# Ansh4121/audio-deepfake-detection-fmsl

Hardware: NVIDIA B200
Metric: utterances/sec (4 s, 16 kHz) LFCC+delta+delta-delta front-end (higher is better)
Workload: dtype f32 (split-fp16 tensor-core DFT, fp32 accumulate)

## Files before the change

### audio-deepfake-detection-fmsl_b200/csrc/fe_gemm_tables.h

```cpp
#ifndef FE_GEMM_TABLES_H_
#define FE_GEMM_TABLES_H_
#include "fe_common.h"

int64_t fe_gemm_plan_layout(const b200fe_params* p, fe_blob_header* h, int64_t off);
int32_t fe_gemm_pack(const b200fe_params* p, fe_blob_header* h, const float* window,
                     const float* fbank, char* base);
bool fe_gemm_variant_built(void);
bool fe_gemm_auto_prefers(const b200fe_params* p);
#endif
```

### audio-deepfake-detection-fmsl_b200/csrc/fe_stream.cu

```cuda
#include <atomic>
#include <stdio.h>
#include <unistd.h>

#include "fe_tc.cuh"

#include "fe_gemm.cuh"
#include "fe_gemm.h"
#include "fe_gemm_tables.h"

namespace {

constexpr int kDrainWarps = 16;
constexpr int kProducerWarp0 = kDrainWarps;
constexpr int kProducerGroups = 2;
constexpr int kProducerWarps = 4 * kProducerGroups;
constexpr int kProducerThreads = kProducerWarps * 32;
constexpr int kMmaWarp0 = kProducerWarp0 + kProducerWarps;
constexpr int kNumMmaWarps = 2;
constexpr int kLoaderWarp = kMmaWarp0 + kNumMmaWarps;
constexpr int kThreads = (kLoaderWarp + 1) * 32;
constexpr int kTileM = FE_GEMM_TILE_M;
constexpr int kMaxSlots = 131;
constexpr int kAStageBytes = 8 * 2 * kTileM * 16;
constexpr int kGmaxStride = (((kMaxSlots + 1) * 4 + 15) & ~15) / 4;

struct stream_args {
  const float* wave;
  const void* tables;
  float* energies;
  unsigned int* group_max;
  int* error_flag;
  int64_t T;
  int64_t row_base;
  int32_t rows, n_frames, n_filter, hop, nhalf, nstages, kpairs;
  int32_t total_frames, tile_frames, n_tiles, top_db_group;
  const int64_t* offsets;
  const int32_t* lengths;
  int64_t flat_rel, dense_rel;
};

__device__ __forceinline__ int64_t row_src(const stream_args& a, int row) {
  if (!a.offsets) return (int64_t)row * a.T;
  const int64_t arow = a.row_base + row;
  const int64_t off = __ldg(a.offsets + arow);
  return fe_clip_in_place(off, __ldg(a.lengths + arow), a.T, a.flat_rel) ? a.flat_rel + off : a.dense_rel + (int64_t)row * a.T;
}

constexpr int kNumBars = 14;

struct smem_layout {
  int samp, a_stage, b_stage, dw, dwn, dctl, dhdr, mid, gmax, us2, midp, exl0, exch, bars, tmem_slot, total;
};

__host__ __device__ inline smem_layout make_layout(int hop, int nhalf, int kpairs) {
  smem_layout L;
  int off = 0;
  L.samp = off;      off += kMaxSlots * hop * 4;
  off = (off + 127) & ~127;
  L.a_stage = off;   off += 2 * kAStageBytes;
  L.b_stage = off;   off += 2 * fe_gemm_b_stage_bytes(nhalf);
  L.dw = off;        off += 2 * (nhalf / 2) * (int)sizeof(fe_drain_w);
  L.dwn = off;       off += 2 * (nhalf / FE_DRAIN_BATCH) * 16 * 4;
  L.dctl = off;      off += (2 * (nhalf / FE_DRAIN_BATCH) * 4 + 15) & ~15;
  L.dhdr = off;      off += (int)sizeof(fe_drain_hdr);
  L.mid = off;       off += kpairs * 4;
  L.gmax = off;      off += 2 * (((kMaxSlots + 1) * 4 + 15) & ~15);
  L.us2 = off;       off += 2 * kTileM * 4;
  L.midp = off;      off += 2 * kProducerGroups * kTileM * 8;
  L.exl0 = off;      off += 2 * 2 * 2 * kTileM * 4;
  L.exch = off;      off += 2 * 2 * kTileM * 4;
  L.bars = off;      off += kNumBars * 8;
  L.tmem_slot = off; off += 16;
  L.total = off;
  return L;
}

enum { BAR_SAMP_FULL = 0, BAR_SAMP_EMPTY = 1, BAR_A_FULL = 2, BAR_B_FULL = 4, BAR_STAGE_FREE = 6, BAR_ACC_FULL = 8,
       BAR_ACC_EMPTY = 9, BAR_PROD_DONE = 10, BAR_SCOUT_FULL = 12, BAR_COUNT = 14 };
static_assert(BAR_COUNT == kNumBars, "barrier count");

#ifdef FE_GEMM_TRACE
#ifndef FE_TRACE_CTA
#define FE_TRACE_CTA 0
#endif
#ifndef FE_TRACE_IT0
#define FE_TRACE_IT0 0
#endif
#define ST_TRACE(ev, it, q) do { if (blockIdx.x == FE_TRACE_CTA && (int)(it) >= FE_TRACE_IT0 && (int)(it) < FE_TRACE_IT0 + 8) { ((long long*)(a.error_flag + 64))[(((int)(it) - FE_TRACE_IT0) * 8 + (q)) * 16 + (ev)] = clock64(); } } while (0)
#else
#define ST_TRACE(ev, it, q) do { } while (0)
#endif

__device__ __forceinline__ uint32_t swz(uint32_t o) { return o ^ (((o >> 7) & 7u) << 4); }

struct tmaps8 {
  CUtensorMap m[8];
};

__device__ __forceinline__ void tma_box_4d(uint32_t dst, const CUtensorMap* map, uint32_t bar, int c0, int c1, int c2, int c3) {
  asm volatile(
      "cp.async.bulk.tensor.4d.shared::cluster.global.mbarrier::complete_tx::bytes [%0], [%1, {%3, %4, %5, %6}], [%2];" ::"r"(dst),
      "l"(map), "r"(bar), "r"(c0), "r"(c1), "r"(c2), "r"(c3)
      : "memory");
}

__device__ __forceinline__ void tma_box_5d(uint32_t dst, const CUtensorMap* map, uint32_t bar, int c0, int c1, int c2, int c3, int c4) {
  asm volatile(
      "cp.async.bulk.tensor.5d.shared::cluster.global.mbarrier::complete_tx::bytes [%0], [%1, {%3, %4, %5, %6, %7}], [%2];" ::"r"(dst),
      "l"(map), "r"(bar), "r"(c0), "r"(c1), "r"(c2), "r"(c3), "r"(c4)
      : "memory");
}
// ... 106 lines not shown
    tmem_ld8(t0 + 2 * tn, se);
    tmem_ld8(t0 + 3 * tn, so);
#endif
    tmem_ld_wait();
    tmem_ld_tie8(ce); tmem_ld_tie8(co); tmem_ld_tie8(se); tmem_ld_tie8(so);
    unsigned ctl;
    asm volatile("ld.shared.u32 %0, [%1];" : "=r"(ctl) : "r"(ctl_addr));
    fe_drain_w w[4];
#pragma unroll
    for (int p = 0; p < 4; ++p)
      asm volatile("ld.shared.v4.f32 {%0, %1, %2, %3}, [%4];" : "=f"(w[p].w[0][0]), "=f"(w[p].w[0][1]), "=f"(w[p].w[1][0]), "=f"(w[p].w[1][1])
                   : "r"(w_addr + 16u * p));
    if (left == 1) {
      tc_fence_before();
      __syncwarp();
      if (lane == 0) mbar_arrive(acc_empty_bar);
    }
    fe_f2 pw[4];
#ifdef FE_EXP_NO_MATH
    st.acc[0].x += ce[0] + co[1] + se[2] + so[3];
    continue;
#endif
#pragma unroll
    for (int p = 0; p < 4; ++p)
      pw[p] = fe_drain_power<RUN>(fe_f2{ce[2 * p], ce[2 * p + 1]}, fe_f2{co[2 * p], co[2 * p + 1]}, fe_f2{se[2 * p], se[2 * p + 1]},
                                  fe_f2{so[2 * p], so[2 * p + 1]});
    fe_drain_batch(pw, w, reinterpret_cast<const float*>(__cvta_shared_to_generic(wn_addr)), ctl, st, emit);
  }
}


// ... 11 lines not shown
    asm volatile("ld.shared.v4.f32 {%0, %1, %2, %3}, [%4];" : "=f"(b.x), "=f"(b.y), "=f"(b.z), "=f"(b.w)
                 : "r"(smem_u32(s_samp) + swz(brow + (hop - j0 - 16) * 4 + ch * 16)));
    buf[4 * ch + 0] = b.x; buf[4 * ch + 1] = b.y; buf[4 * ch + 2] = b.z; buf[4 * ch + 3] = b.w;
  }
  bwd[0] = (j0 == 0) ? fwd[0] : *reinterpret_cast<const float*>(s_samp + swz(brow + (hop - j0) * 4));
#pragma unroll
  for (int i = 1; i < 16; ++i) bwd[i] = buf[16 - i];
  fe_u4 chunk[8];
  fe_stream_produce_unit(fwd, bwd, scale, s_mid + j0, mid_re, mid_im, chunk);
  mbar_wait(bar_stage_free, free_parity, error_flag, 7);
  unsigned char* a_row = a_slot + khalf * kTileM * 16 + m * 16;
#pragma unroll
  for (int sf = 0; sf < 8; ++sf) *reinterpret_cast<fe_u4*>(a_row + sf * fe_gemm_tile_bytes(kTileM)) = chunk[sf];
  fence_proxy_async();
  __syncwarp();
  if (lane == 0) mbar_arrive(bar_a_full);
}

__global__ void __launch_bounds__(kThreads, 1) fe_stream_kernel(const __grid_constant__ tmaps8 maps, const stream_args a) {
  extern __shared__ __align__(1024) unsigned char smem[];
  const smem_layout L = make_layout(a.hop, a.nhalf, a.kpairs);
  const int tid = threadIdx.x, warp = tid >> 5, lane = tid & 31;
  const unsigned char* blob = reinterpret_cast<const unsigned char*>(a.tables);
  const fe_blob_header* h = reinterpret_cast<const fe_blob_header*>(blob);
  const int nF = a.n_frames, hop = a.hop, nfil = a.n_filter;
  const int rs = hop * 4;
  const int npairs = a.nhalf / 2, nbatch = a.nhalf / FE_DRAIN_BATCH;

  if (!h->gemm_ok) {
    if (tid == 0) mbar_timeout(a.error_flag, 98);
    return;
  }
  unsigned char* s_samp = smem + L.samp;
  fe_drain_w* s_dw = reinterpret_cast<fe_drain_w*>(smem + L.dw);
  uint32_t* s_dctl = reinterpret_cast<uint32_t*>(smem + L.dctl);
  float* s_dwn = reinterpret_cast<float*>(smem + L.dwn);
  fe_drain_hdr* s_dhdr = reinterpret_cast<fe_drain_hdr*>(smem + L.dhdr);
  float* s_mid = reinterpret_cast<float*>(smem + L.mid);
  float* s_gmax = reinterpret_cast<float*>(smem + L.gmax);
  float* s_us2 = reinterpret_cast<float*>(smem + L.us2);
  float2* s_midp = reinterpret_cast<float2*>(smem + L.midp);
  float* s_exl0 = reinterpret_cast<float*>(smem + L.exl0);
  float* s_exch = reinterpret_cast<float*>(smem + L.exch);
  uint32_t* s_tmem = reinterpret_cast<uint32_t*>(smem + L.tmem_slot);
  const uint32_t bars = smem_u32(smem + L.bars);
  auto bar = [&](int i) { return bars + 8u * (uint32_t)i; };

  {
    const fe_drain_w* gdw = reinterpret_cast<const fe_drain_w*>(blob + h->off_gemm_dw);
    for (int i = tid; i < 2 * npairs; i += kThreads) s_dw[i] = gdw[i];
    const uint32_t* gctl = reinterpret_cast<const uint32_t*>(blob + h->off_gemm_dctl);
    for (int i = tid; i < 2 * nbatch; i += kThreads) s_dctl[i] = gctl[i];
    const float* gwn = reinterpret_cast<const float*>(blob + h->off_gemm_dwn);
    for (int i = tid; i < 2 * nbatch * 16; i += kThreads) s_dwn[i] = gwn[i];
    const int32_t* ghdr = reinterpret_cast<const int32_t*>(blob + h->off_gemm_dids);
    for (int i = tid; i < (int)(sizeof(fe_drain_hdr) / 4); i += kThreads) reinterpret_cast<int32_t*>(s_dhdr)[i] = ghdr[i];
    const float* gmid = reinterpret_cast<const float*>(blob + h->off_gemm_mid);
    for (int i = tid; i < a.kpairs; i += kThreads) s_mid[i] = (i & 1) ? gmid[a.kpairs + i] : gmid[i];
    float4* z = reinterpret_cast<float4*>(s_samp);
    for (int i = tid; i < kMaxSlots * rs / 16; i += kThreads) z[i] = make_float4(0.f, 0.f, 0.f, 0.f);
    fence_proxy_async();
  }
  if (tid == 0) {
    mbar_init(bar(BAR_SAMP_FULL), 2);
    mbar_init(bar(BAR_SAMP_EMPTY), kProducerWarps);
    mbar_init(bar(BAR_A_FULL + 0), 8);
    mbar_init(bar(BAR_A_FULL + 1), 8);
    mbar_init(bar(BAR_B_FULL + 0), 1);
    mbar_init(bar(BAR_B_FULL + 1), 1);
    mbar_init(bar(BAR_STAGE_FREE + 0), kNumMmaWarps);
    mbar_init(bar(BAR_STAGE_FREE + 1), kNumMmaWarps);
    mbar_init(bar(BAR_ACC_FULL), kNumMmaWarps);
    mbar_init(bar(BAR_ACC_EMPTY), kDrainWarps);
    mbar_init(bar(BAR_PROD_DONE + 0), kProducerWarps);
    mbar_init(bar(BAR_PROD_DONE + 1), kProducerWarps);
    mbar_init(bar(BAR_SCOUT_FULL + 0), kDrainWarps);
    mbar_init(bar(BAR_SCOUT_FULL + 1), kDrainWarps);
    asm volatile("fence.mbarrier_init.release.cluster;" ::: "memory");
  }
  if (warp == kMmaWarp0) {
    asm volatile("tcgen05.alloc.cta_group::1.sync.aligned.shared::cta.b32 [%0], %1;" ::"r"(smem_u32(s_tmem)), "r"(512));
    asm volatile("tcgen05.relinquish_alloc_permit.cta_group::1.sync.aligned;" ::);
  }
  tc_fence_before();
  __syncthreads();
  tc_fence_after();
  const uint32_t tmem_base = *s_tmem;
  const int T = (int)a.T;
  const uint32_t b_stage_bytes = (uint32_t)fe_gemm_b_stage_bytes(a.nhalf);

  if (warp == kLoaderWarp) {
    const unsigned char* gB = blob + h->off_gemm_b;
    const uint32_t row_bytes = (uint32_t)hop * 4u;
    uint32_t n = 0, it = 0;
    for (int tile = blockIdx.x; tile < a.n_tiles; tile += gridDim.x, ++it) {
      const fe_tile_geo g = fe_tile_geometry(tile, a.tile_frames, a.total_frames, nF);
      mbar_wait_relaxed(bar(BAR_SAMP_EMPTY), (it & 1u) ^ 1u, a.error_flag, 1);
      ST_TRACE(0, it, 0);
      int n_edge = 0;
      for (int row = g.row0; row <= g.row_last; ++row) {
        const int sa = row * (nF + 1) - g.sv0, sb = sa + nF;
        n_edge += (sa >= 0 && sa < g.nv) + (sb >= 0 && sb < g.nv);
      }
      fence_proxy_async();
      if (lane == 0) mbar_arrive_expect_tx(bar(BAR_SAMP_FULL), (uint32_t)(g.nv - n_edge) * row_bytes);
      __syncwarp();
      for (int row = g.row0; row <= g.row_last; ++row) {
        const int v_lo = max(g.sv0 - row * (nF + 1), 1), v_hi = min(g.sv0 + g.nv - 1 - row * (nF + 1), nF - 1);
        const int cnt = v_hi - v_lo + 1;
        if (cnt <= 0) continue;
        if (lane < 8 && ((cnt >> lane) & 1)) {
// ... 30 lines not shown
      if (tile + (int)gridDim.x < a.n_tiles) {
        const fe_tile_geo gn = fe_tile_geometry(tile + gridDim.x, a.tile_frames, a.total_frames, nF);
        for (int row = gn.row0; row <= gn.row_last; ++row) {
          const int v_lo = max(gn.sv0 - row * (nF + 1), 1), v_hi = min(gn.sv0 + gn.nv - 1 - row * (nF + 1), nF - 1);
          const int cnt = v_hi - v_lo + 1;
          if (cnt <= 0) continue;
          if (lane < 8 && ((cnt >> lane) & 1)) {
            const int first = cnt & ~((2 << lane) - 1);
            row_prefetch(a, &maps.m[lane], v_lo - 1 + first, row);
          }
        }
      }
      if (lane == 0) {
        for (int q = 0; q < a.nstages; ++q, ++n) {
          const uint32_t s = n & 1u, par = (n >> 1) & 1u;
          mbar_wait_relaxed(bar(BAR_STAGE_FREE + s), par ^ 1u, a.error_flag, 2);
          mbar_arrive_expect_tx(bar(BAR_B_FULL + s), b_stage_bytes);
          bulk_g2s(smem_u32(smem + L.b_stage + s * b_stage_bytes), gB + (size_t)q * b_stage_bytes, b_stage_bytes,
                   bar(BAR_B_FULL + s));
        }
      }
      __syncwarp();
    }
  } else if (warp >= kMmaWarp0) {
    {
      const int sub0 = (4 / kNumMmaWarps) * __shfl_sync(0xffffffffu, warp - kMmaWarp0, 0);
      const uint32_t tmem_u = __shfl_sync(0xffffffffu, tmem_base, 0);
      const uint32_t idesc = (1u << 4) | ((uint32_t)(a.nhalf >> 3) << 17) | ((uint32_t)(kTileM >> 4) << 24);
      const uint32_t b_lbo = (uint32_t)a.nhalf * 16u;
      const uint32_t smem_a = smem_u32(smem + L.a_stage), smem_b = smem_u32(smem + L.b_stage);
      const uint32_t tile_bytes_a = fe_gemm_tile_bytes(kTileM), tile_bytes_b = fe_gemm_tile_bytes(a.nhalf);
      uint32_t n = 0, it = 0;
      for (int tile = blockIdx.x; tile < a.n_tiles; tile += gridDim.x, ++it) {
        mbar_wait_relaxed(bar(BAR_ACC_EMPTY), (it & 1u) ^ 1u, a.error_flag, 3);
        tc_fence_after();
        if (sub0 == 0 && lane == 0) ST_TRACE(8, it, 0);
        for (int q = 0; q < a.nstages; ++q, ++n) {
          const uint32_t s = n & 1u, par = (n >> 1) & 1u;
          mbar_wait_relaxed(bar(BAR_B_FULL + s), par, a.error_flag, 4);
          if (sub0 == 0 && lane == 0) ST_TRACE(10, it, q);
          mbar_wait_relaxed(bar(BAR_A_FULL + s), par, a.error_flag, 5);
          tc_fence_after();
          if (sub0 == 0 && lane == 0) ST_TRACE(3, it, q);
          const uint32_t a_base = smem_a + s * kAStageBytes;
          const uint32_t b_base = smem_b + s * b_stage_bytes;
          if (elect_one()) {
#ifdef FE_EXP_TWO_PRODUCTS
            constexpr int kProducts = 2;
#else
            constexpr int kProducts = 3;
#endif
#pragma unroll
            for (int pr = 0; pr < kProducts; ++pr) {
#pragma unroll
              for (int ds = 0; ds < 4 / kNumMmaWarps; ++ds) {
                const int sub = sub0 + ds;
                const uint64_t da = make_desc(a_base + (2 * sub + (pr == 1 ? 1 : 0)) * tile_bytes_a, kTileM * 16, 128);
                const uint64_t db = make_desc(b_base + (2 * sub + (pr == 2 ? 1 : 0)) * tile_bytes_b, b_lbo, 128);
                umma_f16(tmem_u + (uint32_t)(sub * a.nhalf), da, db, idesc, (q > 0 || pr > 0) ? 1u : 0u);
              }
            }
            umma_commit(bar(BAR_STAGE_FREE + s));
            if (q == a.nstages - 1) umma_commit(bar(BAR_ACC_FULL));
          }
          __syncwarp();
        }
      }
    }
  } else if (warp >= kProducerWarp0) {
    const int pw = warp - kProducerWarp0;
    const int grp = pw >> 2;
    const int quarter = pw & 3;
    const int m = quarter * 32 + lane;
    uint32_t n0 = 0, it = 0;
    for (int tile = blockIdx.x; tile < a.n_tiles; tile += gridDim.x, ++it, n0 += (uint32_t)a.nstages) {
      const fe_tile_geo g = fe_tile_geometry(tile, a.tile_frames, a.total_frames, nF);
      const int mm = min(m, g.count - 1);
      const int row = (g.g0 + mm) / nF;
      const int slot = mm + (row - g.row0);
      const uint32_t tp = it & 1u;
      mbar_wait(bar(BAR_SCOUT_FULL + tp), (it >> 1) & 1u, a.error_flag, 10);
      float scale, unscale;
      {
        const float* gm = s_gmax + tp * kGmaxStride;
        fe_gemm_frame_scale(2.0f * fmaxf(gm[slot], gm[slot + 1]), scale, unscale);
      }
      mbar_wait(bar(BAR_SAMP_FULL), tp, a.error_flag, 6);
      if (tid == kProducerWarp0 * 32) ST_TRACE(1, it, 0);
      if (grp == 0) s_us2[tp * kTileM + m] = unscale * unscale;
      const uint32_t brow = (uint32_t)(slot * rs), frow = brow + (uint32_t)rs;
      float mid_re = 0.0f, mid_im = 0.0f;
#pragma unroll 1
      for (int q = 0; q < a.nstages; ++q) {
        const uint32_t n = n0 + (uint32_t)q, sl = n & 1u, par = (n >> 1) & 1u;
        produce_unit(s_samp, brow, frow, hop, q, grp, m, scale, s_mid, mid_re, mid_im, smem + L.a_stage + sl * kAStageBytes,
                     bar(BAR_STAGE_FREE + sl), par ^ 1u, bar(BAR_A_FULL + sl), a.error_flag, lane);
        if (lane == 0 && quarter == 0) ST_TRACE(2, it, q);
      }
      s_midp[(tp * kProducerGroups + grp) * kTileM + m] = make_float2(mid_re, mid_im);
      __syncwarp();
      if (lane == 0) {
        mbar_arrive(bar(BAR_SAMP_EMPTY));
        mbar_arrive(bar(BAR_PROD_DONE + tp));
      }
    }
  } else {
    const int quarter = warp & 3;
    const int run = (warp >> 2) & 1;
    const int half = warp >> 3;
    const int m = quarter * 32 + lane;
    const fe_drain_w* w_run = s_dw + run * npairs;
    const uint32_t* ctl_run = s_dctl + run * nbatch;
    const float* wn_run = s_dwn + run * nbatch * 16;
    const uint32_t tbase = tmem_base + ((uint32_t)(quarter * 32) << 16);
    const int k_begin = half * (a.nhalf >> 1), k_end = k_begin + (a.nhalf >> 1);
    for (int pre = 0; pre < 2; ++pre) {
      const int tile = blockIdx.x + pre * gridDim.x;
      if (tile < a.n_tiles) {
        const fe_tile_geo g = fe_tile_geometry(tile, a.tile_frames, a.total_frames, nF);
        scout_tile_global(a, nF, hop, g, s_gmax + pre * kGmaxStride, warp, kDrainWarps, lane);
      }
      __syncwarp();
      if (lane == 0) mbar_arrive(bar(BAR_SCOUT_FULL + pre));
    }
    uint32_t it = 0;
    for (int tile = blockIdx.x; tile < a.n_tiles; tile += gridDim.x, ++it) {
      const fe_tile_geo g = fe_tile_geometry(tile, a.tile_frames, a.total_frames, nF);
      const int mm = min(m, g.count - 1);
      const int row = (g.g0 + mm) / nF;
      const int t = (g.g0 + mm) - row * nF;
      const uint32_t tp = it & 1u;
      mbar_wait(bar(BAR_PROD_DONE + tp), (it >> 1) & 1u, a.error_flag, 9);
      emit_store emit;
      emit.base = a.energies;
      emit.off = (uint32_t)((row * nfil) * nF + t);
      emit.n_frames = (uint32_t)nF;
      emit.n_filter = nfil;
      emit.valid = m < g.count;
      emit.us2 = s_us2[tp * kTileM + m];
      emit.vmax = 0.0f;
      float p_mid = 0.0f;
      if (run == 0 && half == 1) {
        const float2 v0 = s_midp[(tp * kProducerGroups + 0) * kTileM + m], v1 = s_midp[(tp * kProducerGroups + 1) * kTileM + m];
        const float bs = (float)(1 << FE_GEMM_B_SCALE_LOG2);
        const float re = (v0.x + v1.x) * bs, im = (v0.y + v1.y) * bs;
        p_mid = fmaf(re, re, im * im);
      }
      fe_drain_state st;
      fe_drain_init(st, *s_dhdr, run, half);
      mbar_wait(bar(BAR_ACC_FULL), tp, a.error_flag, 8);
      tc_fence_after();
      if (lane == 0 && quarter == 0) ST_TRACE(4, it, warp >> 2);
      if (run == 0) drain_walk<0>(tbase, a.nhalf, k_begin, k_end, w_run, ctl_run, wn_run, st, emit, bar(BAR_ACC_EMPTY), lane);
      else drain_walk<1>(tbase, a.nhalf, k_begin, k_end, w_run, ctl_run, wn_run, st, emit, bar(BAR_ACC_EMPTY), lane);
      if (lane == 0 && quarter == 0) ST_TRACE(5, it, warp >> 2);
      float* l0p = s_exl0 + ((tp * 2 + run) * 2) * kTileM + m;
      if (half == 0) {
        l0p[0] = fe_drain_leftover(st, 0, 0.0f, 0.0f);
        l0p[kTileM] = fe_drain_leftover(st, 1, 0.0f, 0.0f);
        quarter_bar(quarter);
      } else {
        quarter_bar(quarter);
        const float l0[2] = {l0p[0], l0p[kTileM]};
        float left[2];
        fe_drain_join_halves(st, *s_dhdr, run, l0, p_mid, left, emit);
        float* ex = s_exch + tp * 2 * kTileM + m;
        if (run == 1) {
          if (s_dhdr->merge[0]) ex[0] = left[0]; else emit(s_dhdr->last[1][0], left[0]);
          if (s_dhdr->merge[1]) ex[kTileM] = left[1]; else emit(s_dhdr->last[1][1], left[1]);
          runs_bar(quarter);
        } else {
          runs_bar(quarter);
          emit(s_dhdr->last[0][0], s_dhdr->merge[0] ? left[0] + ex[0] : left[0]);
          emit(s_dhdr->last[0][1], s_dhdr->merge[1] ? left[1] + ex[kTileM] : left[1]);
        }
      }
      if (a.group_max) {
        const int grp_id = (int)((a.row_base + row) / a.top_db_group);
        const int grp0 = __shfl_sync(0xffffffffu, grp_id, 0);
        if (__all_sync(0xffffffffu, grp_id == grp0)) {
          const unsigned wmax = __reduce_max_sync(0xffffffffu, __float_as_uint(emit.vmax));
          if (lane == 0) atomicMax(a.group_max + grp0, wmax);
        } else if (emit.valid) {
          atomicMax(a.group_max + grp_id, __float_as_uint(emit.vmax));
        }
      }
      if (lane == 0 && quarter == 0) ST_TRACE(6, it, warp >> 2);
      {
        const int tile2 = tile + 2 * (int)gridDim.x;
        if (tile2 < a.n_tiles) {
          const fe_tile_geo g2 = fe_tile_geometry(tile2, a.tile_frames, a.total_frames, nF);
          scout_tile_global(a, nF, hop, g2, s_gmax + tp * kGmaxStride, warp, kDrainWarps, lane);
        }
        __syncwarp();
        if (lane == 0) mbar_arrive(bar(BAR_SCOUT_FULL + tp));
        if (lane == 0 && quarter == 0) ST_TRACE(7, it, warp >> 2);
      }
    }
  }

  tc_fence_before();
  __syncthreads();
  if (warp == kMmaWarp0) {
    asm volatile("tcgen05.dealloc.cta_group::1.sync.aligned.b32 %0, %1;" ::"r"(tmem_base), "r"(512));
  }
}

typedef CUresult (*encode_tiled_fn)(CUtensorMap*, CUtensorMapDataType, cuuint32_t, void*, const cuuint64_t*,
                                    const cuuint64_t*, const cuuint32_t*, const cuuint32_t*, CUtensorMapInterleave,
                                    CUtensorMapSwizzle, CUtensorMapL2promotion, CUtensorMapFloatOOBfill);

encode_tiled_fn get_encode() {
  static std::atomic<encode_tiled_fn> cached{nullptr};
  encode_tiled_fn fn = cached.load(std::memory_order_relaxed);
  if (!fn) {
    void* p = nullptr;
    cudaDriverEntryPointQueryResult q;
    if (cudaGetDriverEntryPoint("cuTensorMapEncodeTiled", &p, cudaEnableDefault, &q) == cudaSuccess &&
        q == cudaDriverEntryPointSuccess) {
      fn = (encode_tiled_fn)p;
      cached.store(fn, std::memory_order_relaxed);
    }
  }
  return fn;
}

}

#ifdef FE_GEMM_TRACE
int* fe_trace_host_flag = nullptr;
#endif
int32_t fe_gemm_compiled(void) { return 1; }

bool fe_gemm_supported(const b200fe_params* p) {
  if (p->n_filter < 1 || p->n_filter > FE_GEMM_MAX_FILTERS) return false;
  if (p->win_length != 2 * p->hop_length || p->win_length > p->n_fft) return false;
  const int kpairs = p->win_length / 2, nhalf = p->n_fft / 4;
  if (kpairs % 32 != 0 || kpairs < 32 || kpairs > 256) return false;
  if (nhalf % 16 != 0 || nhalf < 32 || nhalf > 128) return false;
// ... 38 lines not shown
  a.row_base = row_base;
  a.rows = (int32_t)rows;
  a.n_frames = fa.n_frames;
  a.n_filter = p->n_filter;
  a.hop = p->hop_length;
  a.nhalf = p->n_fft / 4;
  a.kpairs = p->win_length / 2;
  a.nstages = a.kpairs / 32;
  a.total_frames = (int32_t)(rows * fa.n_frames);
  a.tile_frames = fe_tile_frames(fa.n_frames);
  a.n_tiles = (a.total_frames + a.tile_frames - 1) / a.tile_frames;
  a.top_db_group = fa.top_db_group;

  struct map_key {
    const void* base;
    int64_t rows, T;
    int32_t hop, n_frames;
    bool ragged;
    bool operator==(const map_key& o) const { return base == o.base && rows == o.rows && T == o.T && hop == o.hop && n_frames == o.n_frames && ragged == o.ragged; }
  };
  struct map_entry { map_key key; tmaps8 maps; bool valid; };
  constexpr int kMapCache = 8;
  thread_local map_entry cache[kMapCache];
  thread_local int cache_next = 0;
  const map_key key{(const void*)a.wave, rows, fa.T, a.hop, fa.n_frames, in_place};
  const tmaps8* maps_p = nullptr;
  for (int i = 0; i < kMapCache; ++i)
    if (cache[i].valid && cache[i].key == key) { maps_p = &cache[i].maps; break; }
  if (!maps_p) {
    encode_tiled_fn enc = get_encode();
    if (!enc) return cudaErrorNotSupported;
    map_entry& e = cache[cache_next];
    cache_next = (cache_next + 1) % kMapCache;
    e.valid = false;
    const cuuint64_t gdim[5] = {32, (cuuint64_t)(a.hop / 32), (cuuint64_t)(fa.n_frames - 1), in_place ? (cuuint64_t)1 << 31 : (cuuint64_t)rows, 32};
    const cuuint64_t gstride[4] = {128, (cuuint64_t)a.hop * 4, in_place ? (cuuint64_t)16 : (cuuint64_t)fa.T * 4, (cuuint64_t)1 << 35};
    const cuuint32_t estride[5] = {1, 1, 1, 1, 1};
    for (int k = 0; k < 8; ++k) {
      const cuuint32_t box[5] = {32, (cuuint32_t)(a.hop / 32), 1u << k, 1, 1};
      CUresult r = enc(&e.maps.m[k], CU_TENSOR_MAP_DATA_TYPE_FLOAT32, in_place ? 5 : 4, (void*)a.wave, gdim, gstride, box, estride,
                       CU_TENSOR_MAP_INTERLEAVE_NONE, CU_TENSOR_MAP_SWIZZLE_128B, CU_TENSOR_MAP_L2_PROMOTION_L2_128B,
                       CU_TENSOR_MAP_FLOAT_OOB_FILL_NONE);
      if (r != CUDA_SUCCESS) return cudaErrorInvalidValue;
    }
    e.key = key;
    e.valid = true;
    maps_p = &e.maps;
  }
  const int smem = make_layout(a.hop, a.nhalf, a.kpairs).total;
  if (smem > 227 * 1024) return cudaErrorInvalidConfiguration;
  const int dev = fe_current_device();
  if (dev < 0) return cudaErrorInvalidDevice;
  {
    cudaError_t e = fe_ensure_smem((const void*)fe_stream_kernel, (size_t)smem);
    if (e != cudaSuccess) return e;
  }
  const int sms = fe_device_sms(dev);
  const int grid = a.n_tiles < sms ? a.n_tiles : sms;
#ifdef FE_GEMM_TRACE
  {
    static int* host_flag = nullptr;
    extern int* fe_trace_host_flag;
    if (!host_flag) {
      cudaHostAlloc((void**)&host_flag, 256, cudaHostAllocMapped);
      for (int i = 0; i < 64; ++i) host_flag[i] = 0;
      int* dptr = nullptr;
      cudaHostGetDevicePointer((void**)&dptr, host_flag, 0);
      cudaMemcpyToSymbol(g_fe_host_flag, &dptr, sizeof(dptr));
      fe_trace_host_flag = host_flag;
      static struct printer { int* p; ~printer() { fprintf(stderr, "fe_stream timeout codes per warp (code*100000+cta):"); for (int i = 0; i < kThreads / 32; ++i) fprintf(stderr, " w%d:%d", i, p[i]); fprintf(stderr, "\n"); } } pr{host_flag};
    }
  }
  cudaError_t e = cudaMemsetAsync(a.error_flag, 0, 65536, stream);
#else
  cudaError_t e = cudaMemsetAsync(a.error_flag, 0, 4, stream);
#endif
  if (e != cudaSuccess) return e;
  fe_stream_kernel<<<grid, kThreads, smem, stream>>>(*maps_p, a);
  *launches = 1;
  return cudaGetLastError();
}
```

### audio-deepfake-detection-fmsl_b200/csrc/fe_tables.cpp

```cpp
#include <math.h>
#include <stdarg.h>
#include <stdio.h>
#include <string.h>
#include <vector>

#include "fe_common.h"
#include "fe_gemm_tables.h"

static thread_local char g_err[512] = "";

void fe_set_error(const char* fmt, ...) {
  va_list ap;
  va_start(ap, fmt);
  vsnprintf(g_err, sizeof(g_err), fmt, ap);
  va_end(ap);
}

extern "C" const char* b200fe_last_error_string(void) { return g_err; }

extern "C" const char* b200fe_status_string(int32_t s) {
  switch (s) {
    case B200FE_OK: return "ok";
    case B200FE_ERR_BAD_ARG: return "bad argument";
    case B200FE_ERR_UNSUPPORTED: return "unsupported configuration (no CPU fallback)";
// ... 115 lines not shown
    total_w = (int64_t)p->n_filter * n_freq;
    max_len = n_freq;
  }
  h->off_band_w = (int32_t)off;
  h->total_w = (int32_t)total_w;
  h->max_band_len = max_len;
  off = fe_align16(off + (int64_t)p->n_filter * n_freq * 4);
  h->off_dct = (int32_t)off;
  off = fe_align16(off + (int64_t)p->n_filter * (p->n_coef > 0 ? p->n_coef : 0) * 4);
  off = fe_gemm_plan_layout(p, h, off);
  if (off > 0x7fffffff) { fe_set_error("tables blob too large"); return B200FE_ERR_UNSUPPORTED; }
  h->total_bytes = (int32_t)off;
  return B200FE_OK;
}

extern "C" int64_t b200fe_tables_bytes(const b200fe_params* p) {
  int32_t st = fe_validate_params(p);
  if (st != B200FE_OK) return st;
  fe_blob_header h;
  st = plan_layout(p, nullptr, &h, nullptr, nullptr);
  if (st != B200FE_OK) return st;
  return h.total_bytes;
}

extern "C" int32_t b200fe_tables_pack(const b200fe_params* p, const float* window, const float* fbank,
                                      const float* dct, void* blob_host, size_t blob_bytes) {
  int32_t st = fe_validate_params(p);
  if (st != B200FE_OK) return st;
  if (!window || !blob_host) { fe_set_error("window / blob_host is NULL"); return B200FE_ERR_BAD_ARG; }
  if (p->n_filter > 0 && !fbank) { fe_set_error("fbank is NULL but n_filter=%d", p->n_filter); return B200FE_ERR_BAD_ARG; }
// ... 69 lines not shown
```

### audio-deepfake-detection-fmsl_b200/csrc/fe_tc.cuh

```cuda
#ifndef FE_TC_CUH_
#define FE_TC_CUH_
#include <cuda.h>
#include <cuda_runtime.h>
#include <stdint.h>

constexpr uint32_t kSpinLimit = 1u << 21;

__device__ __forceinline__ uint32_t smem_u32(const void* p) { return (uint32_t)__cvta_generic_to_shared(p); }

__device__ __forceinline__ void mbar_init(uint32_t bar, uint32_t count) {
  asm volatile("mbarrier.init.shared::cta.b64 [%0], %1;" ::"r"(bar), "r"(count));
}
__device__ __forceinline__ void mbar_arrive(uint32_t bar) {
  asm volatile("mbarrier.arrive.shared::cta.b64 _, [%0];" ::"r"(bar) : "memory");
}
__device__ __forceinline__ void mbar_arrive_expect_tx(uint32_t bar, uint32_t bytes) {
  asm volatile("mbarrier.arrive.expect_tx.shared::cta.b64 _, [%0], %1;" ::"r"(bar), "r"(bytes) : "memory");
}
__device__ __forceinline__ bool mbar_try_wait(uint32_t bar, uint32_t parity) {
  uint32_t ok;
  asm volatile(
      "{\n\t.reg .pred p;\n\tmbarrier.try_wait.parity.shared::cta.b64 p, [%1], %2, %3;\n\tselp.u32 %0, 1, 0, p;\n\t}\n"
      : "=r"(ok)
      : "r"(bar), "r"(parity), "r"(2000u)
// ... 60 lines not shown
  asm volatile("tcgen05.commit.cta_group::1.mbarrier::arrive::one.shared::cluster.b64 [%0];" ::"r"(bar) : "memory");
}

__device__ __forceinline__ void tma_box_3d(uint32_t dst, const CUtensorMap* map, uint32_t bar, int c0, int c1, int c2) {
  asm volatile(
      "cp.async.bulk.tensor.3d.shared::cluster.global.mbarrier::complete_tx::bytes [%0], [%1, {%3, %4, %5}], [%2];" ::"r"(dst),
      "l"(map), "r"(bar), "r"(c0), "r"(c1), "r"(c2)
      : "memory");
}
__device__ __forceinline__ void bulk_g2s(uint32_t dst, const void* src, uint32_t bytes, uint32_t bar) {
  asm volatile("cp.async.bulk.shared::cluster.global.mbarrier::complete_tx::bytes [%0], [%1], %2, [%3];" ::"r"(dst),
               "l"(src), "r"(bytes), "r"(bar)
               : "memory");
}

__device__ __forceinline__ void tmem_ld16(uint32_t taddr, float* v) {
  uint32_t r[16];
  asm volatile(
      "tcgen05.ld.sync.aligned.32x32b.x16.b32 {%0,%1,%2,%3,%4,%5,%6,%7,%8,%9,%10,%11,%12,%13,%14,%15}, [%16];\n"
      : "=r"(r[0]), "=r"(r[1]), "=r"(r[2]), "=r"(r[3]), "=r"(r[4]), "=r"(r[5]), "=r"(r[6]), "=r"(r[7]), "=r"(r[8]),
        "=r"(r[9]), "=r"(r[10]), "=r"(r[11]), "=r"(r[12]), "=r"(r[13]), "=r"(r[14]), "=r"(r[15])
      : "r"(taddr));
#pragma unroll
  for (int i = 0; i < 16; ++i) v[i] = __uint_as_float(r[i]);
}
__device__ __forceinline__ void tmem_ld8(uint32_t taddr, float* v) {
  uint32_t r[8];
  asm volatile("tcgen05.ld.sync.aligned.32x32b.x8.b32 {%0,%1,%2,%3,%4,%5,%6,%7}, [%8];\n"
               : "=r"(r[0]), "=r"(r[1]), "=r"(r[2]), "=r"(r[3]), "=r"(r[4]), "=r"(r[5]), "=r"(r[6]), "=r"(r[7])
               : "r"(taddr));
// ... 23 lines not shown
```

Measured before the change: 4.481 million.

## Switch DFT GEMM to 2-CTA cluster tcgen05 MMA with split B operand

Launches the streaming kernel as 2-CTA clusters and issues cta_group::2 tcgen05 MMAs with M=256 from the leader CTA. Each CTA loads only half of the B (DFT basis) stage via a paired TMA tensor map, which halves per-CTA B shared-memory traffic and footprint. It also splits the combined stage-free barrier into separate A/B free barriers and adds a third A slot. Cross-CTA barrier arrivals, cluster syncs and dummy tiles for odd tile counts add synchronization complexity, and grid sizing now depends on cluster occupancy.

```diff
diff --git a/audio-deepfake-detection-fmsl_b200/csrc/fe_gemm_tables.h b/audio-deepfake-detection-fmsl_b200/csrc/fe_gemm_tables.h
--- a/audio-deepfake-detection-fmsl_b200/csrc/fe_gemm_tables.h
+++ b/audio-deepfake-detection-fmsl_b200/csrc/fe_gemm_tables.h
@@ -3,6 +3,7 @@
 #include "fe_common.h"
 
 int64_t fe_gemm_plan_layout(const b200fe_params* p, fe_blob_header* h, int64_t off);
+int64_t fe_gemm_b_offset(const b200fe_params* p);
 int32_t fe_gemm_pack(const b200fe_params* p, fe_blob_header* h, const float* window,
                      const float* fbank, char* base);
 bool fe_gemm_variant_built(void);
diff --git a/audio-deepfake-detection-fmsl_b200/csrc/fe_stream.cu b/audio-deepfake-detection-fmsl_b200/csrc/fe_stream.cu
--- a/audio-deepfake-detection-fmsl_b200/csrc/fe_stream.cu
+++ b/audio-deepfake-detection-fmsl_b200/csrc/fe_stream.cu
@@ -34,6 +34,7 @@
   int64_t row_base;
   int32_t rows, n_frames, n_filter, hop, nhalf, nstages, kpairs;
   int32_t total_frames, tile_frames, n_tiles, top_db_group;
+  int32_t b_off;
   const int64_t* offsets;
   const int32_t* lengths;
   int64_t flat_rel, dense_rel;
@@ -46,7 +47,9 @@
   return fe_clip_in_place(off, __ldg(a.lengths + arow), a.T, a.flat_rel) ? a.flat_rel + off : a.dense_rel + (int64_t)row * a.T;
 }
 
-constexpr int kNumBars = 14;
+constexpr int kNumBars = 18;
+constexpr int kASlots = 3;
+constexpr int kBSlots = 2;
 
 struct smem_layout {
   int samp, a_stage, b_stage, dw, dwn, dctl, dhdr, mid, gmax, us2, midp, exl0, exch, bars, tmem_slot, total;
@@ -57,8 +60,8 @@
   int off = 0;
   L.samp = off;      off += kMaxSlots * hop * 4;
   off = (off + 127) & ~127;
-  L.a_stage = off;   off += 2 * kAStageBytes;
-  L.b_stage = off;   off += 2 * fe_gemm_b_stage_bytes(nhalf);
+  L.a_stage = off;   off += kASlots * kAStageBytes;
+  L.b_stage = off;   off += kBSlots * fe_gemm_b_stage_bytes(nhalf) / 2;
   L.dw = off;        off += 2 * (nhalf / 2) * (int)sizeof(fe_drain_w);
   L.dwn = off;       off += 2 * (nhalf / FE_DRAIN_BATCH) * 16 * 4;
   L.dctl = off;      off += (2 * (nhalf / FE_DRAIN_BATCH) * 4 + 15) & ~15;
@@ -75,8 +78,8 @@
   return L;
 }
 
-enum { BAR_SAMP_FULL = 0, BAR_SAMP_EMPTY = 1, BAR_A_FULL = 2, BAR_B_FULL = 4, BAR_STAGE_FREE = 6, BAR_ACC_FULL = 8,
-       BAR_ACC_EMPTY = 9, BAR_PROD_DONE = 10, BAR_SCOUT_FULL = 12, BAR_COUNT = 14 };
+enum { BAR_SAMP_FULL = 0, BAR_SAMP_EMPTY = 1, BAR_A_FULL = 2, BAR_B_FULL = 5, BAR_A_FREE = 7, BAR_B_FREE = 10,
+       BAR_ACC_FULL = 12, BAR_ACC_EMPTY = 13, BAR_PROD_DONE = 14, BAR_SCOUT_FULL = 16, BAR_COUNT = 18 };
 static_assert(BAR_COUNT == kNumBars, "barrier count");
 
 #ifdef FE_GEMM_TRACE
@@ -95,6 +98,7 @@
 
 struct tmaps8 {
   CUtensorMap m[8];
+  CUtensorMap b;
 };
 
 __device__ __forceinline__ void tma_box_4d(uint32_t dst, const CUtensorMap* map, uint32_t bar, int c0, int c1, int c2, int c3) {
@@ -231,7 +235,7 @@
     if (left == 1) {
       tc_fence_before();
       __syncwarp();
-      if (lane == 0) mbar_arrive(acc_empty_bar);
+      if (lane == 0) mbar_arrive_cluster(acc_empty_bar);
     }
     fe_f2 pw[4];
 #ifdef FE_EXP_NO_MATH
@@ -273,7 +277,7 @@
   for (int sf = 0; sf < 8; ++sf) *reinterpret_cast<fe_u4*>(a_row + sf * fe_gemm_tile_bytes(kTileM)) = chunk[sf];
   fence_proxy_async();
   __syncwarp();
-  if (lane == 0) mbar_arrive(bar_a_full);
+  if (lane == 0) mbar_arrive_cluster(bar_a_full);
 }
 
 __global__ void __launch_bounds__(kThreads, 1) fe_stream_kernel(const __grid_constant__ tmaps8 maps, const stream_args a) {
@@ -290,6 +294,11 @@
     if (tid == 0) mbar_timeout(a.error_flag, 98);
     return;
   }
+  if (h->off_gemm_b != a.b_off) {
+    if (tid == 0) mbar_timeout(a.error_flag, 97);
+    return;
+  }
+  const uint32_t rank = cluster_ctarank();
   unsigned char* s_samp = smem + L.samp;
   fe_drain_w* s_dw = reinterpret_cast<fe_drain_w*>(smem + L.dw);
   uint32_t* s_dctl = reinterpret_cast<uint32_t*>(smem + L.dctl);
@@ -304,6 +313,9 @@
   uint32_t* s_tmem = reinterpret_cast<uint32_t*>(smem + L.tmem_slot);
   const uint32_t bars = smem_u32(smem + L.bars);
   auto bar = [&](int i) { return bars + 8u * (uint32_t)i; };
+  auto lead_bar = [&](int i) { return mapa_shared(bar(i), 0); };
+  auto walks = [&](int tile) { return tile - (int)rank < a.n_tiles; };
+  auto geo_tile = [&](int tile) { return min(tile, a.n_tiles - 1); };
 
   {
     const fe_drain_w* gdw = reinterpret_cast<const fe_drain_w*>(blob + h->off_gemm_dw);
@@ -323,14 +335,16 @@
   if (tid == 0) {
     mbar_init(bar(BAR_SAMP_FULL), 2);
     mbar_init(bar(BAR_SAMP_EMPTY), kProducerWarps);
-    mbar_init(bar(BAR_A_FULL + 0), 8);
-    mbar_init(bar(BAR_A_FULL + 1), 8);
-    mbar_init(bar(BAR_B_FULL + 0), 1);
-    mbar_init(bar(BAR_B_FULL + 1), 1);
-    mbar_init(bar(BAR_STAGE_FREE + 0), kNumMmaWarps);
-    mbar_init(bar(BAR_STAGE_FREE + 1), kNumMmaWarps);
+    for (int i = 0; i < kASlots; ++i) {
+      mbar_init(bar(BAR_A_FULL + i), 2 * kProducerWarps);
+      mbar_init(bar(BAR_A_FREE + i), kNumMmaWarps);
+    }
+    for (int i = 0; i < kBSlots; ++i) {
+      mbar_init(bar(BAR_B_FULL + i), 1);
+      mbar_init(bar(BAR_B_FREE + i), kNumMmaWarps);
+    }
     mbar_init(bar(BAR_ACC_FULL), kNumMmaWarps);
-    mbar_init(bar(BAR_ACC_EMPTY), kDrainWarps);
+    mbar_init(bar(BAR_ACC_EMPTY), 2 * kDrainWarps);
     mbar_init(bar(BAR_PROD_DONE + 0), kProducerWarps);
     mbar_init(bar(BAR_PROD_DONE + 1), kProducerWarps);
     mbar_init(bar(BAR_SCOUT_FULL + 0), kDrainWarps);
@@ -338,22 +352,21 @@
     asm volatile("fence.mbarrier_init.release.cluster;" ::: "memory");
   }
   if (warp == kMmaWarp0) {
-    asm volatile("tcgen05.alloc.cta_group::1.sync.aligned.shared::cta.b32 [%0], %1;" ::"r"(smem_u32(s_tmem)), "r"(512));
-    asm volatile("tcgen05.relinquish_alloc_permit.cta_group::1.sync.aligned;" ::);
+    asm volatile("tcgen05.alloc.cta_group::2.sync.aligned.shared::cta.b32 [%0], %1;" ::"r"(smem_u32(s_tmem)), "r"(512));
+    asm volatile("tcgen05.relinquish_alloc_permit.cta_group::2.sync.aligned;" ::);
   }
   tc_fence_before();
-  __syncthreads();
+  cluster_sync();
   tc_fence_after();
   const uint32_t tmem_base = *s_tmem;
   const int T = (int)a.T;
-  const uint32_t b_stage_bytes = (uint32_t)fe_gemm_b_stage_bytes(a.nhalf);
+  const uint32_t b_half_bytes = (uint32_t)fe_gemm_b_stage_bytes(a.nhalf) / 2;
 
   if (warp == kLoaderWarp) {
-    const unsigned char* gB = blob + h->off_gemm_b;
     const uint32_t row_bytes = (uint32_t)hop * 4u;
     uint32_t n = 0, it = 0;
-    for (int tile = blockIdx.x; tile < a.n_tiles; tile += gridDim.x, ++it) {
-      const fe_tile_geo g = fe_tile_geometry(tile, a.tile_frames, a.total_frames, nF);
+    for (int tile = blockIdx.x; walks(tile); tile += gridDim.x, ++it) {
+      const fe_tile_geo g = fe_tile_geometry(geo_tile(tile), a.tile_frames, a.total_frames, nF);
       mbar_wait_relaxed(bar(BAR_SAMP_EMPTY), (it & 1u) ^ 1u, a.error_flag, 1);
       ST_TRACE(0, it, 0);
       int n_edge = 0;
@@ -414,36 +427,35 @@
       if (lane == 0) {
         for (int q = 0; q < a.nstages; ++q, ++n) {
           const uint32_t s = n & 1u, par = (n >> 1) & 1u;
-          mbar_wait_relaxed(bar(BAR_STAGE_FREE + s), par ^ 1u, a.error_flag, 2);
-          mbar_arrive_expect_tx(bar(BAR_B_FULL + s), b_stage_bytes);
-          bulk_g2s(smem_u32(smem + L.b_stage + s * b_stage_bytes), gB + (size_t)q * b_stage_bytes, b_stage_bytes,
-                   bar(BAR_B_FULL + s));
+          mbar_wait_relaxed(bar(BAR_B_FREE + s), par ^ 1u, a.error_flag, 2);
+          if (rank == 0) mbar_arrive_expect_tx(bar(BAR_B_FULL + s), 2u * b_half_bytes);
+          tma_box_3d_pair(smem_u32(smem + L.b_stage + s * b_half_bytes), &maps.b, lead_bar(BAR_B_FULL + s), 0, (int)rank, 16 * q);
         }
       }
       __syncwarp();
     }
   } else if (warp >= kMmaWarp0) {
-    {
+    if (rank == 0) {
       const int sub0 = (4 / kNumMmaWarps) * __shfl_sync(0xffffffffu, warp - kMmaWarp0, 0);
       const uint32_t tmem_u = __shfl_sync(0xffffffffu, tmem_base, 0);
-      const uint32_t idesc = (1u << 4) | ((uint32_t)(a.nhalf >> 3) << 17) | ((uint32_t)(kTileM >> 4) << 24);
-      const uint32_t b_lbo = (uint32_t)a.nhalf * 16u;
+      const uint32_t idesc = (1u << 4) | ((uint32_t)(a.nhalf >> 3) << 17) | ((uint32_t)(2 * kTileM >> 4) << 24);
+      const uint32_t b_lbo = (uint32_t)a.nhalf * 8u;
       const uint32_t smem_a = smem_u32(smem + L.a_stage), smem_b = smem_u32(smem + L.b_stage);
-      const uint32_t tile_bytes_a = fe_gemm_tile_bytes(kTileM), tile_bytes_b = fe_gemm_tile_bytes(a.nhalf);
+      const uint32_t tile_bytes_a = fe_gemm_tile_bytes(kTileM), tile_bytes_b = fe_gemm_tile_bytes(a.nhalf / 2);
       uint32_t n = 0, it = 0;
-      for (int tile = blockIdx.x; tile < a.n_tiles; tile += gridDim.x, ++it) {
-        mbar_wait_relaxed(bar(BAR_ACC_EMPTY), (it & 1u) ^ 1u, a.error_flag, 3);
+      for (int tile = blockIdx.x; walks(tile); tile += gridDim.x, ++it) {
+        mbar_wait_cluster(bar(BAR_ACC_EMPTY), (it & 1u) ^ 1u, a.error_flag, 11);
         tc_fence_after();
         if (sub0 == 0 && lane == 0) ST_TRACE(8, it, 0);
         for (int q = 0; q < a.nstages; ++q, ++n) {
-          const uint32_t s = n & 1u, par = (n >> 1) & 1u;
-          mbar_wait_relaxed(bar(BAR_B_FULL + s), par, a.error_flag, 4);
+          const uint32_t sb = n & 1u, pb = (n >> 1) & 1u, sa = n % kASlots, pa = (n / kASlots) & 1u;
+          mbar_wait_cluster(bar(BAR_B_FULL + sb), pb, a.error_flag, 12);
           if (sub0 == 0 && lane == 0) ST_TRACE(10, it, q);
-          mbar_wait_relaxed(bar(BAR_A_FULL + s), par, a.error_flag, 5);
+          mbar_wait_cluster(bar(BAR_A_FULL + sa), pa, a.error_flag, 13);
           tc_fence_after();
           if (sub0 == 0 && lane == 0) ST_TRACE(3, it, q);
-          const uint32_t a_base = smem_a + s * kAStageBytes;
-          const uint32_t b_base = smem_b + s * b_stage_bytes;
+          const uint32_t a_base = smem_a + sa * kAStageBytes;
+          const uint32_t b_base = smem_b + sb * b_half_bytes;
           if (elect_one()) {
 #ifdef FE_EXP_TWO_PRODUCTS
             constexpr int kProducts = 2;
@@ -457,11 +469,12 @@
                 const int sub = sub0 + ds;
                 const uint64_t da = make_desc(a_base + (2 * sub + (pr == 1 ? 1 : 0)) * tile_bytes_a, kTileM * 16, 128);
                 const uint64_t db = make_desc(b_base + (2 * sub + (pr == 2 ? 1 : 0)) * tile_bytes_b, b_lbo, 128);
-                umma_f16(tmem_u + (uint32_t)(sub * a.nhalf), da, db, idesc, (q > 0 || pr > 0) ? 1u : 0u);
+                umma_f16_pair(tmem_u + (uint32_t)(sub * a.nhalf), da, db, idesc, (q > 0 || pr > 0) ? 1u : 0u);
               }
             }
-            umma_commit(bar(BAR_STAGE_FREE + s));
-            if (q == a.nstages - 1) umma_commit(bar(BAR_ACC_FULL));
+            umma_commit_pair(bar(BAR_A_FREE + sa), 3);
+            umma_commit_pair(bar(BAR_B_FREE + sb), 3);
+            if (q == a.nstages - 1) umma_commit_pair(bar(BAR_ACC_FULL), 3);
           }
           __syncwarp();
         }
@@ -473,8 +486,8 @@
     const int quarter = pw & 3;
     const int m = quarter * 32 + lane;
     uint32_t n0 = 0, it = 0;
-    for (int tile = blockIdx.x; tile < a.n_tiles; tile += gridDim.x, ++it, n0 += (uint32_t)a.nstages) {
-      const fe_tile_geo g = fe_tile_geometry(tile, a.tile_frames, a.total_frames, nF);
+    for (int tile = blockIdx.x; walks(tile); tile += gridDim.x, ++it, n0 += (uint32_t)a.nstages) {
+      const fe_tile_geo g = fe_tile_geometry(geo_tile(tile), a.tile_frames, a.total_frames, nF);
       const int mm = min(m, g.count - 1);
       const int row = (g.g0 + mm) / nF;
       const int slot = mm + (row - g.row0);
@@ -492,9 +505,9 @@
       float mid_re = 0.0f, mid_im = 0.0f;
 #pragma unroll 1
       for (int q = 0; q < a.nstages; ++q) {
-        const uint32_t n = n0 + (uint32_t)q, sl = n & 1u, par = (n >> 1) & 1u;
+        const uint32_t n = n0 + (uint32_t)q, sl = n % kASlots, par = (n / kASlots) & 1u;
         produce_unit(s_samp, brow, frow, hop, q, grp, m, scale, s_mid, mid_re, mid_im, smem + L.a_stage + sl * kAStageBytes,
-                     bar(BAR_STAGE_FREE + sl), par ^ 1u, bar(BAR_A_FULL + sl), a.error_flag, lane);
+                     bar(BAR_A_FREE + sl), par ^ 1u, lead_bar(BAR_A_FULL + sl), a.error_flag, lane);
         if (lane == 0 && quarter == 0) ST_TRACE(2, it, q);
       }
       s_midp[(tp * kProducerGroups + grp) * kTileM + m] = make_float2(mid_re, mid_im);
@@ -516,16 +529,18 @@
     const int k_begin = half * (a.nhalf >> 1), k_end = k_begin + (a.nhalf >> 1);
     for (int pre = 0; pre < 2; ++pre) {
       const int tile = blockIdx.x + pre * gridDim.x;
-      if (tile < a.n_tiles) {
-        const fe_tile_geo g = fe_tile_geometry(tile, a.tile_frames, a.total_frames, nF);
+      if (walks(tile)) {
+        const fe_tile_geo g = fe_tile_geometry(geo_tile(tile), a.tile_frames, a.total_frames, nF);
         scout_tile_global(a, nF, hop, g, s_gmax + pre * kGmaxStride, warp, kDrainWarps, lane);
       }
       __syncwarp();
       if (lane == 0) mbar_arrive(bar(BAR_SCOUT_FULL + pre));
     }
+    const uint32_t acc_empty = lead_bar(BAR_ACC_EMPTY);
     uint32_t it = 0;
-    for (int tile = blockIdx.x; tile < a.n_tiles; tile += gridDim.x, ++it) {
-      const fe_tile_geo g = fe_tile_geometry(tile, a.tile_frames, a.total_frames, nF);
+    for (int tile = blockIdx.x; walks(tile); tile += gridDim.x, ++it) {
+      const bool real = tile < a.n_tiles;
+      const fe_tile_geo g = fe_tile_geometry(geo_tile(tile), a.tile_frames, a.total_frames, nF);
       const int mm = min(m, g.count - 1);
       const int row = (g.g0 + mm) / nF;
       const int t = (g.g0 + mm) - row * nF;
@@ -536,7 +551,7 @@
       emit.off = (uint32_t)((row * nfil) * nF + t);
       emit.n_frames = (uint32_t)nF;
       emit.n_filter = nfil;
-      emit.valid = m < g.count;
+      emit.valid = real && m < g.count;
       emit.us2 = s_us2[tp * kTileM + m];
       emit.vmax = 0.0f;
       float p_mid = 0.0f;
@@ -551,8 +566,8 @@
       mbar_wait(bar(BAR_ACC_FULL), tp, a.error_flag, 8);
       tc_fence_after();
       if (lane == 0 && quarter == 0) ST_TRACE(4, it, warp >> 2);
-      if (run == 0) drain_walk<0>(tbase, a.nhalf, k_begin, k_end, w_run, ctl_run, wn_run, st, emit, bar(BAR_ACC_EMPTY), lane);
-      else drain_walk<1>(tbase, a.nhalf, k_begin, k_end, w_run, ctl_run, wn_run, st, emit, bar(BAR_ACC_EMPTY), lane);
+      if (run == 0) drain_walk<0>(tbase, a.nhalf, k_begin, k_end, w_run, ctl_run, wn_run, st, emit, acc_empty, lane);
+      else drain_walk<1>(tbase, a.nhalf, k_begin, k_end, w_run, ctl_run, wn_run, st, emit, acc_empty, lane);
       if (lane == 0 && quarter == 0) ST_TRACE(5, it, warp >> 2);
       float* l0p = s_exl0 + ((tp * 2 + run) * 2) * kTileM + m;
       if (half == 0) {
@@ -575,7 +590,7 @@
           emit(s_dhdr->last[0][1], s_dhdr->merge[1] ? left[1] + ex[kTileM] : left[1]);
         }
       }
-      if (a.group_max) {
+      if (a.group_max && real) {
         const int grp_id = (int)((a.row_base + row) / a.top_db_group);
         const int grp0 = __shfl_sync(0xffffffffu, grp_id, 0);
         if (__all_sync(0xffffffffu, grp_id == grp0)) {
@@ -588,8 +603,8 @@
       if (lane == 0 && quarter == 0) ST_TRACE(6, it, warp >> 2);
       {
         const int tile2 = tile + 2 * (int)gridDim.x;
-        if (tile2 < a.n_tiles) {
-          const fe_tile_geo g2 = fe_tile_geometry(tile2, a.tile_frames, a.total_frames, nF);
+        if (walks(tile2)) {
+          const fe_tile_geo g2 = fe_tile_geometry(geo_tile(tile2), a.tile_frames, a.total_frames, nF);
           scout_tile_global(a, nF, hop, g2, s_gmax + tp * kGmaxStride, warp, kDrainWarps, lane);
         }
         __syncwarp();
@@ -600,9 +615,9 @@
   }
 
   tc_fence_before();
-  __syncthreads();
+  cluster_sync();
   if (warp == kMmaWarp0) {
-    asm volatile("tcgen05.dealloc.cta_group::1.sync.aligned.b32 %0, %1;" ::"r"(tmem_base), "r"(512));
+    asm volatile("tcgen05.dealloc.cta_group::2.sync.aligned.b32 %0, %1;" ::"r"(tmem_base), "r"(512));
   }
 }
 
@@ -623,6 +638,29 @@
     }
   }
   return fn;
+}
+
+int fe_stream_max_clusters(int dev, int smem) {
+  static std::atomic<int> cache[kFeMaxDevices];
+  if (dev >= 0 && dev < kFeMaxDevices) {
+    const int c = cache[dev].load(std::memory_order_relaxed);
+    if (c > 0) return c;
+  }
+  cudaLaunchConfig_t cfg = {};
+  cfg.gridDim = dim3(2 * (unsigned)fe_device_sms(dev));
+  cfg.blockDim = dim3(kThreads);
+  cfg.dynamicSmemBytes = (size_t)smem;
+  cudaLaunchAttribute attr[1];
+  attr[0].id = cudaLaunchAttributeClusterDimension;
+  attr[0].val.clusterDim.x = 2;
+  attr[0].val.clusterDim.y = 1;
+  attr[0].val.clusterDim.z = 1;
+  cfg.attrs = attr;
+  cfg.numAttrs = 1;
+  int n = 0;
+  if (cudaOccupancyMaxActiveClusters(&n, (const void*)fe_stream_kernel, &cfg) != cudaSuccess || n < 1) return 0;
+  if (dev < kFeMaxDevices) cache[dev].store(n, std::memory_order_relaxed);
+  return n;
 }
 
 }
@@ -691,19 +729,23 @@
 
   struct map_key {
     const void* base;
+    const void* tables;
     int64_t rows, T;
-    int32_t hop, n_frames;
+    int32_t hop, n_frames, n_fft, win, n_filter, n_coef;
     bool ragged;
-    bool operator==(const map_key& o) const { return base == o.base && rows == o.rows && T == o.T && hop == o.hop && n_frames == o.n_frames && ragged == o.ragged; }
+    bool operator==(const map_key& o) const {
+      return base == o.base && tables == o.tables && rows == o.rows && T == o.T && hop == o.hop && n_frames == o.n_frames &&
+             n_fft == o.n_fft && win == o.win && n_filter == o.n_filter && n_coef == o.n_coef && ragged == o.ragged;
+    }
   };
-  struct map_entry { map_key key; tmaps8 maps; bool valid; };
+  struct map_entry { map_key key; tmaps8 maps; int32_t b_off; bool valid; };
   constexpr int kMapCache = 8;
   thread_local map_entry cache[kMapCache];
   thread_local int cache_next = 0;
-  const map_key key{(const void*)a.wave, rows, fa.T, a.hop, fa.n_frames, in_place};
+  const map_key key{(const void*)a.wave, fa.tables, rows, fa.T, a.hop, fa.n_frames, p->n_fft, p->win_length, p->n_filter, p->n_coef, in_place};
   const tmaps8* maps_p = nullptr;
   for (int i = 0; i < kMapCache; ++i)
-    if (cache[i].valid && cache[i].key == key) { maps_p = &cache[i].maps; break; }
+    if (cache[i].valid && cache[i].key == key) { maps_p = &cache[i].maps; a.b_off = cache[i].b_off; break; }
   if (!maps_p) {
     encode_tiled_fn enc = get_encode();
     if (!enc) return cudaErrorNotSupported;
@@ -720,6 +762,20 @@
                        CU_TENSOR_MAP_FLOAT_OOB_FILL_NONE);
       if (r != CUDA_SUCCESS) return cudaErrorInvalidValue;
     }
+    const int64_t b_off = fe_gemm_b_offset(p);
+    if (b_off < 0) return cudaErrorInvalidValue;
+    {
+      const cuuint64_t bdim[3] = {(cuuint64_t)a.nhalf * 2, 2, (cuuint64_t)a.nstages * 16};
+      const cuuint64_t bstride[2] = {(cuuint64_t)a.nhalf * 8, (cuuint64_t)a.nhalf * 16};
+      const cuuint32_t bbox[3] = {(cuuint32_t)a.nhalf * 2, 1, 16};
+      const cuuint32_t bestride[3] = {1, 1, 1};
+      CUresult r = enc(&e.maps.b, CU_TENSOR_MAP_DATA_TYPE_UINT32, 3, (void*)((const char*)fa.tables + b_off), bdim, bstride, bbox,
+                       bestride, CU_TENSOR_MAP_INTERLEAVE_NONE, CU_TENSOR_MAP_SWIZZLE_NONE, CU_TENSOR_MAP_L2_PROMOTION_L2_256B,
+                       CU_TENSOR_MAP_FLOAT_OOB_FILL_NONE);
+      if (r != CUDA_SUCCESS) return cudaErrorInvalidValue;
+    }
+    e.b_off = (int32_t)b_off;
+    a.b_off = e.b_off;
     e.key = key;
     e.valid = true;
     maps_p = &e.maps;
@@ -732,8 +788,10 @@
     cudaError_t e = fe_ensure_smem((const void*)fe_stream_kernel, (size_t)smem);
     if (e != cudaSuccess) return e;
   }
-  const int sms = fe_device_sms(dev);
-  const int grid = a.n_tiles < sms ? a.n_tiles : sms;
+  const int clusters = fe_stream_max_clusters(dev, smem);
+  if (clusters < 1) return cudaErrorInvalidConfiguration;
+  const int n_pairs = (a.n_tiles + 1) / 2;
+  const int grid = 2 * (n_pairs < clusters ? n_pairs : clusters);
 #ifdef FE_GEMM_TRACE
   {
     static int* host_flag = nullptr;
@@ -753,7 +811,20 @@
   cudaError_t e = cudaMemsetAsync(a.error_flag, 0, 4, stream);
 #endif
   if (e != cudaSuccess) return e;
-  fe_stream_kernel<<<grid, kThreads, smem, stream>>>(*maps_p, a);
+  cudaLaunchConfig_t cfg = {};
+  cfg.gridDim = dim3((unsigned)grid);
+  cfg.blockDim = dim3(kThreads);
+  cfg.dynamicSmemBytes = (size_t)smem;
+  cfg.stream = stream;
+  cudaLaunchAttribute attr[1];
+  attr[0].id = cudaLaunchAttributeClusterDimension;
+  attr[0].val.clusterDim.x = 2;
+  attr[0].val.clusterDim.y = 1;
+  attr[0].val.clusterDim.z = 1;
+  cfg.attrs = attr;
+  cfg.numAttrs = 1;
+  e = cudaLaunchKernelEx(&cfg, fe_stream_kernel, *maps_p, a);
+  if (e != cudaSuccess) return e;
   *launches = 1;
   return cudaGetLastError();
 }
diff --git a/audio-deepfake-detection-fmsl_b200/csrc/fe_tables.cpp b/audio-deepfake-detection-fmsl_b200/csrc/fe_tables.cpp
--- a/audio-deepfake-detection-fmsl_b200/csrc/fe_tables.cpp
+++ b/audio-deepfake-detection-fmsl_b200/csrc/fe_tables.cpp
@@ -153,6 +153,12 @@
   return B200FE_OK;
 }
 
+int64_t fe_gemm_b_offset(const b200fe_params* p) {
+  fe_blob_header h;
+  if (fe_validate_params(p) != B200FE_OK || plan_layout(p, nullptr, &h, nullptr, nullptr) != B200FE_OK || !h.gemm_ok) return -1;
+  return h.off_gemm_b;
+}
+
 extern "C" int64_t b200fe_tables_bytes(const b200fe_params* p) {
   int32_t st = fe_validate_params(p);
   if (st != B200FE_OK) return st;
diff --git a/audio-deepfake-detection-fmsl_b200/csrc/fe_tc.cuh b/audio-deepfake-detection-fmsl_b200/csrc/fe_tc.cuh
--- a/audio-deepfake-detection-fmsl_b200/csrc/fe_tc.cuh
+++ b/audio-deepfake-detection-fmsl_b200/csrc/fe_tc.cuh
@@ -98,6 +98,55 @@
                : "memory");
 }
 
+__device__ __forceinline__ uint32_t cluster_ctarank() {
+  uint32_t r;
+  asm volatile("mov.u32 %0, %%cluster_ctarank;" : "=r"(r));
+  return r;
+}
+__device__ __forceinline__ void cluster_sync() {
+  asm volatile("barrier.cluster.arrive.release.aligned;\n\tbarrier.cluster.wait.acquire.aligned;" ::: "memory");
+}
+__device__ __forceinline__ uint32_t mapa_shared(uint32_t addr, uint32_t rank) {
+  uint32_t r;
+  asm volatile("mapa.shared::cluster.u32 %0, %1, %2;" : "=r"(r) : "r"(addr), "r"(rank));
+  return r;
+}
+__device__ __forceinline__ void mbar_arrive_cluster(uint32_t cbar) {
+  asm volatile("mbarrier.arrive.release.cluster.shared::cluster.b64 _, [%0];" ::"r"(cbar) : "memory");
+}
+__device__ __forceinline__ void mbar_wait_cluster(uint32_t bar, uint32_t parity, int* error_flag, int code) {
+#pragma unroll 1
+  for (uint32_t spin = 0; spin < kSpinLimit; ++spin) {
+    uint32_t ok;
+    asm volatile(
+        "{\n\t.reg .pred p;\n\tmbarrier.try_wait.parity.acquire.cluster.shared::cta.b64 p, [%1], %2, %3;\n\tselp.u32 %0, 1, 0, p;\n\t}\n"
+        : "=r"(ok)
+        : "r"(bar), "r"(parity), "r"(2000u)
+        : "memory");
+    if (ok) return;
+    __nanosleep(128);
+  }
+  mbar_timeout(error_flag, code);
+}
+__device__ __forceinline__ void umma_f16_pair(uint32_t tmem_d, uint64_t da, uint64_t db, uint32_t idesc, uint32_t accumulate) {
+  asm volatile(
+      "{\n\t.reg .pred p;\n\tsetp.ne.b32 p, %4, 0;\n\t"
+      "tcgen05.mma.cta_group::2.kind::f16 [%0], %1, %2, %3, p;\n\t}\n" ::"r"(tmem_d),
+      "l"(da), "l"(db), "r"(idesc), "r"(accumulate)
+      : "memory");
+}
+__device__ __forceinline__ void umma_commit_pair(uint32_t bar, uint16_t mask) {
+  asm volatile("tcgen05.commit.cta_group::2.mbarrier::arrive::one.shared::cluster.multicast::cluster.b64 [%0], %1;" ::"r"(bar),
+               "h"(mask)
+               : "memory");
+}
+__device__ __forceinline__ void tma_box_3d_pair(uint32_t dst, const CUtensorMap* map, uint32_t cbar, int c0, int c1, int c2) {
+  asm volatile(
+      "cp.async.bulk.tensor.3d.cta_group::2.shared::cluster.global.mbarrier::complete_tx::bytes [%0], [%1, {%3, %4, %5}], [%2];" ::"r"(dst),
+      "l"(map), "r"(cbar), "r"(c0), "r"(c1), "r"(c2)
+      : "memory");
+}
+
 __device__ __forceinline__ void tmem_ld16(uint32_t taddr, float* v) {
   uint32_t r[16];
   asm volatile(
```

Result: slower. 3.965 million, median of 6 (-11.5%).
